# SuperScientificSoftwareLaboratory/PanguLU

Hardware: AMD Instinct MI355X
Metric: numeric factorisation GFLOP/s (pangulu_gstrf, R64) (higher is better)
Workload: dtype f64

## Files before the change

pangulu_amd/csrc/platform/pg_hip_backend.h:

```cpp
#pragma once

struct DiagAux
{
    u32 *d_cp = nullptr;
    u16 *d_ri = nullptr;
    u32 *d_vi = nullptr;
    u32 nnz = 0;
    u32 brow = 0;
};

struct Ring
{
    static const int NSEG = 32;
    std::vector<int> pending;
    size_t seg_bytes = 0;
    char *h = nullptr, *d = nullptr;
    hipEvent_t ev[NSEG];
    bool used[NSEG];
    int cur = 0;
};

struct EventPair
{
    hipEvent_t a, b;
    int cls;
    int split_cls;
    double split_frac;
    unsigned long long tag[3];
};

#define PG_FLOP_WORDS 48

struct Backend
{
    bool ready = false;
    int device = 0;
    hipStream_t stream = nullptr;
    bool bulk_streams_masked = false;
    hipStream_t stream2 = nullptr;
    hipStream_t stream3 = nullptr;
    hipEvent_t ev_fork = nullptr, ev_join = nullptr, ev_fork3 = nullptr, ev_join3 = nullptr;
    hipStream_t stream_front = nullptr;
    hipEvent_t ev_front_fork = nullptr, ev_front_join = nullptr;
    long long opt_front_fork = 1;
    bool getrf_join_pending = false;
    hipStream_t stream_rec = nullptr;
    hipEvent_t ev_rec_fork = nullptr, ev_rec = nullptr;
    std::atomic<bool> rec_dirty{false};
    hipStream_t stream_bg = nullptr;
    hipEvent_t ev_bg_fork = nullptr, ev_bg_done = nullptr;
    hipStream_t stream_early = nullptr;
    bool bg_active = false;
    std::unordered_set<const void *> bg_tiles;
    long long opt_background_updates = 1;
    long long opt_front_stages = 2;
    long long opt_front_min_wgs = 2048;
    long long opt_front_unit = 1;
    long long opt_tiles_stages = 2;
    long long opt_tiles_unit = 1;
    unsigned long long front_workgroups = 0, general_workgroups = 0;
    long long opt_records_stream = 1;
    int nb_cfg = 0;
    unsigned long long generation = 0;
    long long opt_host_mirror = 1;
    long long opt_dense_permille = 2;
    long long opt_profile = 0;
    long long opt_assume_independent = 0;
    long long opt_getrf_strict = 0;
    long long opt_count_flops = 1;
    long long opt_group_chunk = 8;
    long long opt_small_launch_tasks = 2048;
    long long opt_trsm_dense_permille = 5;
    long long opt_two_streams = 1;
    double mfma_flops_executed = 0;
    Ring ring;
    unsigned *d_progress = nullptr;
    size_t progress_next = 0;
    unsigned long long chase_launches = 0, chase_solves = 0;
    unsigned long long zgetrf_tasks = 0;
    unsigned long long *d_flops = nullptr;
    val_t *getrf_scratch = nullptr;
    int getrf_scratch_slots = 0;
    std::unordered_map<const void *, DiagAux> diag_aux;
    pangulu_hip_stats_t stats;
    std::vector<EventPair> pending_events;
    std::vector<hipEvent_t> event_pool;
    std::mutex mutex;
};

Backend B;

struct Recorder
{
    int mode = 0;
    bool valid = false;
    const void *owner = nullptr;
    unsigned long long signature = 0;
    std::vector<std::function<void()>> ops;
    std::vector<std::function<void()>> prologue;
    bool in_prologue = false;
    std::vector<hipEvent_t> early_events;
    struct Seg
    {
        char *h, *d, *twin;
        size_t cap;
    };
    std::vector<Seg> segs;
    size_t descriptor_bytes = 0;
    bool pack = false;
    struct Tail
    {
        int seg;
        size_t used;
    };
    std::vector<Tail> tails;
    int nb = 0;
    unsigned long long generation = 0;
    pangulu_hip_stats_t stats_before, stats_delta;
    unsigned long long wgs_before[4] = {0, 0, 0, 0}, wgs_delta[4] = {0, 0, 0, 0};
};
Recorder REC;

#define PROGRESS_WORDS 8192
struct PendingGetrf
{
    bool active = false, hold = false;
    int nb = 0;
    size_t take = 0;
    const void *d_tasks = nullptr;
    unsigned *d_progress = nullptr;
    std::vector<const double *> images;
    std::function<void()> plain;
    std::function<void()> post;
};
PendingGetrf PEND;
inline void flush_pending_getrf()
{
    if (!PEND.active || PEND.hold)
        return;
    PEND.active = false;
    PEND.plain();
    PEND.post();
    PEND.plain = nullptr;
    PEND.post = nullptr;
}

inline void flush_pending_getrf_locked();

template <class T>
inline T rec_xl(T v)
{
    if constexpr (std::is_pointer<T>::value)
    {
        const char *p = reinterpret_cast<const char *>(v);
        for (const Recorder::Seg &sg : REC.segs)
            if (p >= sg.d && p < sg.d + sg.cap)
                return reinterpret_cast<T>(const_cast<char *>(sg.twin + (p - sg.d)));
    }
    return v;
}

template <class K, class... A>
inline void pg_launch(K kernel, dim3 grid, dim3 block, size_t shmem, hipStream_t st, A... args)
{
    flush_pending_getrf();
    if (REC.mode != 0)
    {
        auto targs = std::make_tuple(rec_xl(args)...);
        (REC.in_prologue ? REC.prologue : REC.ops).emplace_back([=]()
                             { std::apply([&](auto... a)
                                          { hipLaunchKernelGGL(kernel, grid, block, (unsigned)shmem, st, a...); },
                                          targs); });
        if (REC.mode == 2)
            return;
    }
    hipLaunchKernelGGL(kernel, grid, block, (unsigned)shmem, st, args...);
}
#define PG_LAUNCH(kernel_, grid_, block_, shmem_, stream_, ...) pg_launch(kernel_, grid_, block_, shmem_, stream_, __VA_ARGS__)

inline void pg_event_record(hipEvent_t e, hipStream_t s)
{
    flush_pending_getrf();
    if (REC.mode != 0)
        (REC.in_prologue ? REC.prologue : REC.ops).emplace_back([e, s]() { HIP_CHECK(hipEventRecord(e, s)); });
    if (REC.mode != 2)
        HIP_CHECK(hipEventRecord(e, s));
}
inline void pg_stream_wait(hipStream_t s, hipEvent_t e)
{
    flush_pending_getrf();
    if (REC.mode != 0)
        REC.ops.emplace_back([e, s]() { HIP_CHECK(hipStreamWaitEvent(s, e, 0)); });
    if (REC.mode != 2)
        HIP_CHECK(hipStreamWaitEvent(s, e, 0));
}

inline void flush_pending_getrf_locked()
{
    if (!PEND.active)
        return;
    std::lock_guard<std::mutex> g(B.mutex);
    flush_pending_getrf();
}

void ensure_ready()
{
    if (B.ready)
        return;
    int ndev = 0;
    hipError_t e = hipGetDeviceCount(&ndev);
    if (e != hipSuccess || ndev <= 0)
    {
        fprintf(stderr, "[PanguLU-AMD ERROR] no HIP device available (%s); the GPU_HIP platform has no CPU fallback\n",
                e == hipSuccess ? "device count is 0" : hipGetErrorString(e));
        exit(EXIT_FAILURE);
    }
    HIP_CHECK(hipSetDevice(B.device));
    {
        long reserved = 0;
        if (const char *e = getenv("PANGULU_HIP_RESERVED_CUS"))
            reserved = atol(e);
        hipDeviceProp_t prop;
        HIP_CHECK(hipGetDeviceProperties(&prop, B.device));
        const int ncu = prop.multiProcessorCount;
        if (reserved > 0 && reserved < ncu / 2 && ncu % 32 == 0)
        {
            std::vector<uint32_t> mask((size_t)ncu / 32, 0xFFFFFFFFu);
            for (int i = ncu - (int)reserved; i < ncu; i++)
                mask[(size_t)i / 32] &= ~(1u << (i % 32));
            HIP_CHECK(hipExtStreamCreateWithCUMask(&B.stream, (uint32_t)mask.size(), mask.data()));
            HIP_CHECK(hipExtStreamCreateWithCUMask(&B.stream2, (uint32_t)mask.size(), mask.data()));
            B.bulk_streams_masked = true;
        }
        else
        {
            HIP_CHECK(hipStreamCreateWithFlags(&B.stream, hipStreamNonBlocking));
            HIP_CHECK(hipStreamCreateWithFlags(&B.stream2, hipStreamNonBlocking));
        }
    }
    HIP_CHECK(hipStreamCreateWithFlags(&B.stream_front, hipStreamNonBlocking));
    HIP_CHECK(hipEventCreateWithFlags(&B.ev_front_fork, hipEventDisableTiming));
    HIP_CHECK(hipEventCreateWithFlags(&B.ev_front_join, hipEventDisableTiming));
    if (const char *e = getenv("PANGULU_HIP_FRONT_FORK"))
        B.opt_front_fork = atol(e);
    HIP_CHECK(hipEventCreateWithFlags(&B.ev_fork, hipEventDisableTiming));
    HIP_CHECK(hipEventCreateWithFlags(&B.ev_join, hipEventDisableTiming));
    HIP_CHECK(hipStreamCreateWithFlags(&B.stream3, hipStreamNonBlocking));
    HIP_CHECK(hipEventCreateWithFlags(&B.ev_fork3, hipEventDisableTiming));
    HIP_CHECK(hipEventCreateWithFlags(&B.ev_join3, hipEventDisableTiming));
    HIP_CHECK(hipStreamCreateWithFlags(&B.stream_rec, hipStreamNonBlocking));
    HIP_CHECK(hipEventCreateWithFlags(&B.ev_rec_fork, hipEventDisableTiming));
    HIP_CHECK(hipEventCreateWithFlags(&B.ev_rec, hipEventDisableTiming));
    if (const char *e = getenv("PANGULU_HIP_RECORDS_STREAM"))
        B.opt_records_stream = atol(e);
    HIP_CHECK(hipStreamCreateWithFlags(&B.stream_early, hipStreamNonBlocking));
    HIP_CHECK(hipStreamCreateWithFlags(&B.stream_bg, hipStreamNonBlocking));
    HIP_CHECK(hipEventCreateWithFlags(&B.ev_bg_fork, hipEventDisableTiming));
    HIP_CHECK(hipEventCreateWithFlags(&B.ev_bg_done, hipEventDisableTiming));
    if (const char *e = getenv("PANGULU_HIP_BACKGROUND_UPDATES"))
        B.opt_background_updates = atol(e);
    if (const char *e = getenv("PANGULU_HIP_FRONT_STAGES"))
        B.opt_front_stages = atol(e);
    if (const char *e = getenv("PANGULU_HIP_FRONT_UNIT"))
        B.opt_front_unit = atol(e);
    if (const char *e = getenv("PANGULU_HIP_FRONT_MIN_WGS"))
        B.opt_front_min_wgs = atol(e);
    if (const char *e = getenv("PANGULU_HIP_TILES_STAGES"))
        B.opt_tiles_stages = atol(e);
    if (const char *e = getenv("PANGULU_HIP_GROUP_CHUNK"))
        B.opt_group_chunk = atol(e);
    if (const char *e = getenv("PANGULU_HIP_TILES_UNIT"))
        B.opt_tiles_unit = atol(e);
    if (const char *e = getenv("PANGULU_HIP_DENSE_PERMILLE"))
        B.opt_dense_permille = atol(e);
    if (const char *e = getenv("PANGULU_HIP_TRSM_DENSE_PERMILLE"))
        B.opt_trsm_dense_permille = atol(e);
    if (const char *e = getenv("PANGULU_HIP_SMALL_LAUNCH_TASKS"))
        B.opt_small_launch_tasks = atol(e);
    B.ring.seg_bytes = (size_t)8 << 20;
    HIP_CHECK(hipHostMalloc((void **)&B.ring.h, B.ring.seg_bytes * Ring::NSEG, hipHostMallocNonCoherent | hipHostMallocMapped));
    HIP_CHECK(hipHostGetDevicePointer((void **)&B.ring.d, B.ring.h, 0));
    for (int i = 0; i < Ring::NSEG; i++)
    {
        HIP_CHECK(hipEventCreateWithFlags(&B.ring.ev[i], hipEventDisableTiming));
        B.ring.used[i] = false;
    }
    HIP_CHECK(hipMalloc((void **)&B.d_flops, sizeof(unsigned long long) * PG_FLOP_WORDS));
    HIP_CHECK(hipMemset(B.d_flops, 0, sizeof(unsigned long long) * PG_FLOP_WORDS));
    memset(&B.stats, 0, sizeof(B.stats));
    B.ready = true;
}

struct Segment
{
    char *h, *d;
    size_t cap, used;
    int index;
    int rec_idx = -1;
    size_t rec_off = 0;
    template <typename T>
    T *alloc(size_t count, T **dev)
    {
        size_t off = (used + 15) & ~(size_t)15;
        if (off + sizeof(T) * count > cap)
            return nullptr;
        used = off + sizeof(T) * count;
        *dev = reinterpret_cast<T *>(d + off);
        return reinterpret_cast<T *>(h + off);
    }
};

double g_host_seconds[6] = {0, 0, 0, 0, 0, 0};
struct HostTimer
{
    int k;
    std::chrono::steady_clock::time_point t0;
    explicit HostTimer(int k_) : k(k_), t0(std::chrono::steady_clock::now()) {}
    ~HostTimer() { g_host_seconds[k] += std::chrono::duration<double>(std::chrono::steady_clock::now() - t0).count(); }
};

void release_pending_segments(hipStream_t on = nullptr)
{
    Ring &r = B.ring;
    for (int i : r.pending)
    {
        HIP_CHECK(hipEventRecord(r.ev[i], on ? on : B.stream));
        r.used[i] = true;
    }
    r.pending.clear();
}

void join_records(hipStream_t s)
{
    if (!B.rec_dirty.load(std::memory_order_acquire))
        return;
    pg_stream_wait(s, B.ev_rec);
    if (s == B.stream)
        B.rec_dirty.store(false, std::memory_order_release);
}

void join_background(hipStream_t s)
{
    if (!B.bg_active)
        return;
    pg_stream_wait(s, B.ev_bg_done);
    if (s == B.stream)
    {
        B.bg_active = false;
        B.bg_tiles.clear();
    }
}

Segment acquire_segment(size_t want = 0)
{
    Ring &r = B.ring;
    if (REC.mode != 0)
    {
        const size_t min_room = want ? std::min(r.seg_bytes, (want + 4096 + 65535) & ~(size_t)65535) : ((size_t)2 << 20);
        for (size_t k = REC.tails.size(); k-- > 0;)
        {
            const Recorder::Tail t = REC.tails[k];
            const Recorder::Seg &sg = REC.segs[(size_t)t.seg];
            if (sg.cap - t.used < min_room)
                continue;
            REC.tails.erase(REC.tails.begin() + (long)k);
            Segment s;
            s.h = sg.h + t.used;
            s.d = sg.d + t.used;
            s.cap = sg.cap - t.used;
            s.used = 0;
            s.index = -2;
            s.rec_idx = t.seg;
            s.rec_off = t.used;
            return s;
        }
        const size_t bytes = std::min(r.seg_bytes, std::max(min_room, (size_t)4 << 20));
        char *h = nullptr, *d = nullptr, *twin = nullptr;
        HIP_CHECK(hipHostMalloc((void **)&h, bytes, hipHostMallocNonCoherent | hipHostMallocMapped));
        HIP_CHECK(hipHostGetDevicePointer((void **)&d, h, 0));
        HIP_CHECK(hipMalloc((void **)&twin, bytes));
        REC.segs.push_back(Recorder::Seg{h, d, twin, bytes});
        REC.descriptor_bytes += bytes;
        Segment s;
        s.h = h;
        s.d = d;
        s.cap = bytes;
        s.used = 0;
        s.index = -2;
        s.rec_idx = (int)REC.segs.size() - 1;
        s.rec_off = 0;
        return s;
    }
    int i = r.cur;
    r.cur = (r.cur + 1) % Ring::NSEG;
    if (r.used[i])
    {
        HostTimer ht(4);
        HIP_CHECK(hipEventSynchronize(r.ev[i]));
    }
    Segment s;
    s.h = r.h + (size_t)i * r.seg_bytes;
    s.d = r.d + (size_t)i * r.seg_bytes;
    s.cap = r.seg_bytes;
    s.used = 0;
    s.index = i;
    return s;
}

void commit_segment(Segment &s)
{
    if (s.index >= 0)
        B.ring.pending.push_back(s.index);
    else if (s.index == -2 && REC.mode != 0)
    {
        const size_t used = s.rec_off + ((s.used + 255) & ~(size_t)255);
        if (used + ((size_t)64 << 10) <= REC.segs[(size_t)s.rec_idx].cap)
            REC.tails.push_back(Recorder::Tail{s.rec_idx, used});
    }
}
// ... 177 lines not shown
```

pangulu_amd/csrc/platform/pg_hip_front.h:

```cpp
#pragma once

#define FR_TILE 128
#define FR_KS 16
#define FR_LDA 144
#define FR_STAGE_DOUBLES (FR_KS * FR_LDA + FR_TILE * FR_KS)
#define FR_THREADS 512

typedef const char __attribute__((address_space(1))) *fr_gptr;
typedef void __attribute__((address_space(3))) *fr_lptr;

template <int STAGES, bool PREFETCH>
__global__ __launch_bounds__(FR_THREADS, (STAGES <= 2 ? 4 : 2)) void ssssm_front_f64_kernel(const SsssmTaskD *__restrict__ tasks, int nb, const SsssmWorkD *__restrict__ work,
                                                                     unsigned long long *__restrict__ product_counter, unsigned unit)
{
    __shared__ __align__(16) double lds[STAGES * FR_STAGE_DOUBLES];
    const int tiles = nb / FR_TILE;
    const unsigned bid = logical_block_id(unit ? unit : (unsigned)(tiles * tiles));
    const SsssmWorkD G = work[bid];
    const int tile = (int)G.tile;
    const int tid = threadIdx.x, lane = tid & 63;
    const int wave = __builtin_amdgcn_readfirstlane(tid >> 6);
    const int M0 = (tile % tiles) * FR_TILE, N0 = (tile / tiles) * FR_TILE;
    const int wm = (wave & 1) * 64, wn = (wave >> 1) * 32;
    const int l15 = lane & 15, l4 = lane >> 4;
    const int ntask = (int)(G.task_end - G.task_begin);
    const int steps_shift = nb == 256 ? 4 : 3;
    const int steps_per_task = 1 << steps_shift;
    const int T = ntask << steps_shift;
    const SsssmTaskD *my_tasks = tasks + G.task_begin;

    const unsigned a_voff = (unsigned)lane * 16u;
    const int bc = lane >> 3, bj = lane & 7;
    unsigned b_voff[2];
#pragma unroll
    for (int par = 0; par < 2; par++)
        b_voff[par] = ((unsigned)bc * (unsigned)nb + 2u * (unsigned)(bj ^ ((4 * par + (bc >> 1)) & 7))) * 8u;

    auto issue = [&](int st)
    {
        const int t = st >> steps_shift, k0 = (st & (steps_per_task - 1)) * FR_KS;
        const fr_gptr pa = (fr_gptr)reinterpret_cast<const char *>(my_tasks[t].a.val);
        const fr_gptr pb = (fr_gptr)reinterpret_cast<const char *>(my_tasks[t].b.val);
        double *stage = lds + (st % STAGES) * FR_STAGE_DOUBLES;
#pragma unroll
        for (int h = 0; h < 2; h++)
        {
            const int k = wave + 8 * h;
            const fr_gptr src = dg_scalar_base(pa + ((size_t)(k0 + k) * nb + M0) * 8) + a_voff;
            __builtin_amdgcn_global_load_lds((const void __attribute__((address_space(1))) *)src, (fr_lptr)(stage + k * FR_LDA), 16, 0, 0);
        }
#pragma unroll
        for (int h = 0; h < 2; h++)
        {
            const int g = wave + 8 * h;
            const fr_gptr src = dg_scalar_base(pb + ((size_t)(N0 + 8 * g) * nb + k0) * 8) + b_voff[wave & 1];
            __builtin_amdgcn_global_load_lds((const void __attribute__((address_space(1))) *)src, (fr_lptr)(stage + FR_KS * FR_LDA + g * 128), 16, 0, 0);
        }
    };

    double __attribute__((address_space(1))) *C = (double __attribute__((address_space(1))) *)reinterpret_cast<double *>(G.cdense);
    const unsigned c_voff = ((unsigned)l4 * (unsigned)nb + (unsigned)l15) * 8u;
#define FR_C(ni_, mi_, r_)                                                                           \
    (*(double __attribute__((address_space(1))) *)(dg_scalar_base((const char __attribute__((address_space(1))) *)C +                    \
                                                                  ((size_t)(N0 + wn + (ni_) * 16 + 4 * (r_)) * nb + M0 + wm) * 8) + \
                                                   dg_lane_offset(c_voff) + (mi_) * 128))
#ifndef FR_PRELOAD
#define FR_PRELOAD 1
#endif
    const bool preload = FR_PRELOAD && !G.atomic && T > 0;
    v4f64 acc[2][4];
#pragma unroll
    for (int ni = 0; ni < 2; ni++)
#pragma unroll
        for (int mi = 0; mi < 4; mi++)
        {
            if (preload)
            {
#pragma unroll
                for (int r = 0; r < 4; r++)
                    acc[ni][mi][r] = FR_C(ni, mi, r);
            }
            else
                acc[ni][mi] = (v4f64){0.0, 0.0, 0.0, 0.0};
        }

#pragma unroll
    for (int p = 0; p < STAGES - 1; p++)
        if (p < T)
            issue(p);

    const int a_frag = l4 * FR_LDA + wm + l15;
    int b_frag[2][2];
#pragma unroll
    for (int ni = 0; ni < 2; ni++)
    {
        const int n = wn + ni * 16 + l15;
        b_frag[ni][0] = FR_KS * FR_LDA + n * 16 + (l4 & 1);
        b_frag[ni][1] = (n >> 1) & 7;
    }

    for (int st = 0; st < T; st++)
    {
        const int ahead = min(STAGES - 2, T - 1 - st);
        if (STAGES >= 4 && ahead >= 2)
            asm volatile("s_waitcnt vmcnt(8)" ::: "memory");
        else if (STAGES >= 3 && ahead >= 1)
            asm volatile("s_waitcnt vmcnt(4)" ::: "memory");
        else
            asm volatile("s_waitcnt vmcnt(0)" ::: "memory");
        __builtin_amdgcn_s_barrier();
        if (st + STAGES - 1 < T)
            issue(st + STAGES - 1);
        const double *sA = lds + (st % STAGES) * FR_STAGE_DOUBLES;
#if PG_PLANES > 1
        const bool add = my_tasks[st >> steps_shift].sign < 0;
#endif
#if PG_PLANES > 1
#define FR_MFMA(ni_, mi_, fb_, fa_)                                                                                        \
    if (add)                                                                                                                \
        acc[ni_][mi_] = __builtin_amdgcn_mfma_f64_16x16x4f64(fb_, fa_, acc[ni_][mi_], 0, 0, 0);                          \
    else                                                                                                                    \
        acc[ni_][mi_] = __builtin_amdgcn_mfma_f64_16x16x4f64(fb_, fa_, acc[ni_][mi_], 0, 0, DG_NEG_A);
#else
#define FR_MFMA(ni_, mi_, fb_, fa_) acc[ni_][mi_] = __builtin_amdgcn_mfma_f64_16x16x4f64(fb_, fa_, acc[ni_][mi_], 0, 0, DG_NEG_A);
#endif
#define FR_READ(fa_, fb_, kq_)                                                                        \
    {                                                                                                 \
        _Pragma("unroll") for (int mi = 0; mi < 4; mi++)(fa_)[mi] = sA[a_frag + (kq_) * 4 * FR_LDA + mi * 16]; \
        _Pragma("unroll") for (int ni = 0; ni < 2; ni++)(fb_)[ni] = sA[b_frag[ni][0] + 2 * ((2 * (kq_) + (l4 >> 1)) ^ b_frag[ni][1])]; \
    }
        if (PREFETCH)
        {
            double fa[2][4], fb[2][2];
            FR_READ(fa[0], fb[0], 0)
#pragma unroll
            for (int kq = 0; kq < FR_KS / 4; kq++)
            {
                if (kq + 1 < FR_KS / 4)
                    FR_READ(fa[(kq + 1) & 1], fb[(kq + 1) & 1], kq + 1)
#pragma unroll
                for (int ni = 0; ni < 2; ni++)
#pragma unroll
                    for (int mi = 0; mi < 4; mi++)
                    {
                        FR_MFMA(ni, mi, fb[kq & 1][ni], fa[kq & 1][mi])
                    }
            }
        }
        else
        {
#pragma unroll
            for (int kq = 0; kq < FR_KS / 4; kq++)
            {
                double fa[4], fb[2];
                FR_READ(fa, fb, kq)
#pragma unroll
                for (int ni = 0; ni < 2; ni++)
#pragma unroll
                    for (int mi = 0; mi < 4; mi++)
                    {
                        FR_MFMA(ni, mi, fb[ni], fa[mi])
                    }
            }
        }
#undef FR_READ
#undef FR_MFMA
    }
    if (product_counter && lane == 0 && T)
        atomicAdd(product_counter, (unsigned long long)(8 * T));

    if (preload)
    {
#pragma unroll
        for (int ni = 0; ni < 2; ni++)
#pragma unroll
            for (int mi = 0; mi < 4; mi++)
#pragma unroll
                for (int r = 0; r < 4; r++)
                    FR_C(ni, mi, r) = acc[ni][mi][r];
        return;
    }
#pragma unroll
    for (int ni = 0; ni < 2; ni++)
    {
        if (G.atomic)
        {
#pragma unroll
            for (int mi = 0; mi < 4; mi++)
#pragma unroll
                for (int r = 0; r < 4; r++)
                    atomicAdd((double *)&FR_C(ni, mi, r), acc[ni][mi][r]);
            continue;
        }
        double old[4][4];
#pragma unroll
        for (int mi = 0; mi < 4; mi++)
#pragma unroll
            for (int r = 0; r < 4; r++)
                old[mi][r] = FR_C(ni, mi, r);
#pragma unroll
        for (int mi = 0; mi < 4; mi++)
#pragma unroll
            for (int r = 0; r < 4; r++)
                FR_C(ni, mi, r) = old[mi][r] + acc[ni][mi][r];
    }
#undef FR_C
}

#define TL_WINDOW 16
#ifndef TL_MARK
#define TL_PROBE_DECL
#define TL_MARK(i)
#define TL_PROBE_STEP
#define TL_PROBE_FLUSH
#endif
#ifndef TL_ITEM
#define TL_ITEM_DECL
#define TL_ITEM(i)
#define TL_ITEM_COUNT
#endif
#define TV_STEPS (TL_WINDOW * 16)
__global__ __launch_bounds__(FR_THREADS, 4) void ssssm_tilesv_f64_kernel(const SsssmTaskD *__restrict__ tasks, int nb, const SsssmWorkD *__restrict__ work,
                                                                          unsigned long long *__restrict__ product_counter, unsigned unit)
{
    __shared__ __align__(16) double lds[2 * FR_STAGE_DOUBLES];
    __shared__ unsigned long long s_spa[TV_STEPS], s_spb[TV_STEPS];
    __shared__ u32 s_step[TV_STEPS];
    __shared__ u32 s_cnt[FR_THREADS / 64];
#if PG_PLANES > 1
    __shared__ double s_sign[TL_WINDOW];
#endif
    const int tiles = nb / FR_TILE;
    const unsigned bid = logical_block_id(unit ? unit : (unsigned)(tiles * tiles));
    const SsssmWorkD G = work[bid];
    const int tile = (int)G.tile;
    const int tid = threadIdx.x, lane = tid & 63;
    const int wave = __builtin_amdgcn_readfirstlane(tid >> 6);
    const int M0 = (tile % tiles) * FR_TILE, N0 = (tile / tiles) * FR_TILE;
    const int wr = wave & 1, wc = wave >> 1;
    const int l15 = lane & 15, l4 = lane >> 4;
    const int ntask = (int)(G.task_end - G.task_begin);
    const int nslab = nb / FR_KS;
    const SsssmTaskD *my_tasks = tasks + G.task_begin;

    const unsigned a_voff = (unsigned)lane * 16u;
    const int a_piece = lane >> 3;
    const int bc = lane >> 3, bj = lane & 7;
    const unsigned b_voff = ((unsigned)bc * (unsigned)nb + 2u * (unsigned)(bj ^ ((4 * (wave & 1) + (bc >> 1)) & 7))) * 8u;

    v4f64 acc[2][4];
#pragma unroll
    for (int ni = 0; ni < 2; ni++)
#pragma unroll
        for (int mi = 0; mi < 4; mi++)
            acc[ni][mi] = (v4f64){0.0, 0.0, 0.0, 0.0};
    unsigned touched = 0, nprod = 0;

    const int a_frag = l4 * FR_LDA + wr * 16 + l15;
    int b_frag[2][2];
#pragma unroll
    for (int ni = 0; ni < 2; ni++)
    {
        const int n = (wc + 4 * ni) * 16 + l15;
        b_frag[ni][0] = FR_KS * FR_LDA + n * 16 + (l4 & 1);
        b_frag[ni][1] = (n >> 1) & 7;
    }
    const bool all_live = G.pad_ != 0;
    const int slab_shift = nb == 256 ? 4 : 3;

    auto uniform64 = [&](unsigned long long v) -> fr_gptr
    { return (fr_gptr)(((unsigned long long)(unsigned)__builtin_amdgcn_readfirstlane((int)(v >> 32)) << 32) | (unsigned)__builtin_amdgcn_readfirstlane((int)v)); };
    auto issue = [&](unsigned w, fr_gptr pa, fr_gptr pb, int stage_no)
    {
        const unsigned ab = w & 0xFFu, bb = (w >> 8) & 0xFFu;
        const int k0 = (int)((w >> 16) & 15u) * FR_KS;
        double *stage = lds + stage_no * FR_STAGE_DOUBLES;
        const bool a_live = (ab >> a_piece) & 1u;
#pragma unroll
        for (int h = 0; h < 2; h++)
        {
            const int k = wave + 8 * h;
            const unsigned off = a_live ? (unsigned)(((k0 + k) * nb + M0) * 8) + a_voff : 0u;
            __builtin_amdgcn_global_load_lds((const void __attribute__((address_space(1))) *)(dg_scalar_base(pa) + off), (fr_lptr)(stage + k * FR_LDA), 16, 0, 0);
        }
#pragma unroll
        for (int h = 0; h < 2; h++)
        {
            const int g = wave + 8 * h;
            if (!((bb >> (g >> 1)) & 1u))
                continue;
            const unsigned off = (unsigned)(((N0 + 8 * g) * nb + k0) * 8) + b_voff;
            __builtin_amdgcn_global_load_lds((const void __attribute__((address_space(1))) *)(dg_scalar_base(pb) + off), (fr_lptr)(stage + FR_KS * FR_LDA + g * 128), 16, 0, 0);
        }
    };

    double __attribute__((address_space(1))) *C = (double __attribute__((address_space(1))) *)reinterpret_cast<double *>(G.cdense);
    const unsigned c_voff = ((unsigned)l4 * (unsigned)nb + (unsigned)l15) * 8u;
#define TL_C(ni_, mi_, r_)                                                                           \
    (*(double __attribute__((address_space(1))) *)(dg_scalar_base((const char __attribute__((address_space(1))) *)C +                    \
                                                                  ((size_t)(N0 + (wc + 4 * (ni_)) * 16 + 4 * (r_)) * nb + M0 + wr * 16) * 8) + \
                                                   dg_lane_offset(c_voff) + (mi_) * 256))
    unsigned pre = 0;
    const bool may_preload = !G.atomic && ntask <= TL_WINDOW;

    int stage_head = 0;
    TL_ITEM_DECL
    TL_ITEM_COUNT
    for (int win0 = 0; win0 < ntask; win0 += TL_WINDOW)
    {
        __syncthreads();
        int T;
        if (all_live)
        {
            T = min(TL_WINDOW, ntask - win0) * nslab;
            if (tid < T)
            {
                const int t_ = tid >> slab_shift;
                const SsssmTaskD &Tm = my_tasks[win0 + t_];
                s_step[tid] = ((unsigned)t_ << 20) | ((unsigned)(tid & (nslab - 1)) << 16) | 0xFFFFu;
                s_spa[tid] = (unsigned long long)reinterpret_cast<const double *>(Tm.a.val);
                s_spb[tid] = (unsigned long long)reinterpret_cast<const double *>(Tm.b.val);
#if PG_PLANES > 1
                if ((tid & (nslab - 1)) == 0)
                    s_sign[t_] = Tm.sign;
#endif
            }
            __syncthreads();
        }
        else
        {
            unsigned v = 0;
            unsigned long long pa_v = 0, pb_v = 0;
            const int t_ = tid >> 4, s_ = tid & 15;
            if (tid < TL_WINDOW * 16 && win0 + t_ < ntask && s_ < nslab)
            {
                const SsssmTaskD &Tm = my_tasks[win0 + t_];
                const double *pa_ = reinterpret_cast<const double *>(Tm.a.val), *pb_ = reinterpret_cast<const double *>(Tm.b.val);
                pa_v = (unsigned long long)pa_;
                pb_v = (unsigned long long)pb_;
                unsigned ab_, bb_ = 0;
                if (Tm.has_map)
                {
                    ab_ = ((unsigned)Tm.amap[s_] >> (M0 / 16)) & 0xFFu;
                    bb_ = ((unsigned)Tm.bmap_t[s_] >> (N0 / 16)) & 0xFFu;
                }
                else
                {
                    ab_ = ((unsigned)mirror_map(pa_, nb)[s_] >> (M0 / 16)) & 0xFFu;
                    const uint4 mb_ = *reinterpret_cast<const uint4 *>(mirror_map(pb_, nb) + N0 / 16);
                    const unsigned w_[4] = {mb_.x, mb_.y, mb_.z, mb_.w};
#pragma unroll
                    for (int c_ = 0; c_ < 8; c_++)
                        bb_ |= (((w_[c_ >> 1] >> (16 * (c_ & 1))) >> s_) & 1u) << c_;
                }
                if (ab_ && bb_ && (!G.slab_mask || ((G.slab_mask >> s_) & 1u)))
                    v = (bb_ << 8) | ab_ | ((unsigned)s_ << 16) | ((unsigned)t_ << 20);
#if PG_PLANES > 1
                if (s_ == 0)
                    s_sign[t_] = Tm.sign;
#endif
            }
            const unsigned long long bal = __ballot(v != 0);
            TL_ITEM(0)
            if (lane == 0)
                s_cnt[wave] = (u32)__builtin_popcountll(bal);
            __syncthreads();
            unsigned at = (unsigned)__builtin_popcountll(bal & ((1ull << lane) - 1ull)), all = 0;
#pragma unroll
            for (int w_i = 0; w_i < FR_THREADS / 64; w_i++)
            {
                const unsigned c_ = s_cnt[w_i];
                at += w_i < wave ? c_ : 0u;
                all += c_;
            }
            if (v)
            {
                s_step[at] = v;
                s_spa[at] = pa_v;
                s_spb[at] = pb_v;
            }
            __syncthreads();
            T = __builtin_amdgcn_readfirstlane((int)all);
            TL_ITEM(1)
        }
        if (T == 0)
            continue;

        if (may_preload)
        {
            unsigned m = 0;
            if (all_live)
                m = 0xFFu;
            else
            {
                for (int e = lane; e < T; e += 64)
                {
                    const unsigned w = s_step[e];
                    const unsigned ab = w & 0xFFu, bb = (w >> 8) & 0xFFu;
                    const unsigned a4 = ((ab >> wr) & 1u) | (((ab >> (2 + wr)) & 1u) << 1) | (((ab >> (4 + wr)) & 1u) << 2) | (((ab >> (6 + wr)) & 1u) << 3);
                    if ((bb >> wc) & 1u)
                        m |= a4;
                    if ((bb >> (wc + 4)) & 1u)
                        m |= a4 << 4;
                }
#pragma unroll
                for (int off = 32; off > 0; off >>= 1)
                    m |= (unsigned)__shfl_xor((int)m, off, 64);
            }
            pre = (unsigned)__builtin_amdgcn_readfirstlane((int)m);
#pragma unroll
            for (int ni = 0; ni < 2; ni++)
#pragma unroll
                for (int mi = 0; mi < 4; mi++)
                    if ((pre >> (4 * ni + mi)) & 1u)
                    {
#pragma unroll
                        for (int r = 0; r < 4; r++)
                            acc[ni][mi][r] = TL_C(ni, mi, r);
                    }
        }
        TL_ITEM(2)
        unsigned wC = (unsigned)__builtin_amdgcn_readfirstlane((int)s_step[0]), wN = 0;
        fr_gptr paN = uniform64(s_spa[0]), pbN = uniform64(s_spb[0]);
        issue(wC, paN, pbN, stage_head);
        TL_ITEM(3)
        if (T > 1)
        {
            wN = (unsigned)__builtin_amdgcn_readfirstlane((int)s_step[1]);
            paN = uniform64(s_spa[1]);
            pbN = uniform64(s_spb[1]);
        }
        TL_PROBE_DECL
        for (int st = 0; st < T; st++)
        {
            TL_MARK(6)
            TL_PROBE_STEP
            const int e2 = min(st + 2, T - 1);
            const unsigned v_w = s_step[e2];
            const unsigned long long v_pa = s_spa[e2], v_pb = s_spb[e2];
            asm volatile("s_waitcnt vmcnt(0)" ::: "memory");
            TL_MARK(0)
            __builtin_amdgcn_s_barrier();
            TL_MARK(1)
            const unsigned w2 = (unsigned)__builtin_amdgcn_readfirstlane((int)v_w);
            const fr_gptr pa2 = uniform64(v_pa), pb2 = uniform64(v_pb);
            const double *sA = lds + ((stage_head + st) & 1) * FR_STAGE_DOUBLES;
            const unsigned ab = wC & 0xFFu, bb = (wC >> 8) & 0xFFu;
            const unsigned a4 = ((ab >> wr) & 1u) | (((ab >> (2 + wr)) & 1u) << 1) | (((ab >> (4 + wr)) & 1u) << 2) | (((ab >> (6 + wr)) & 1u) << 3);
            const unsigned b2 = ((bb >> wc) & 1u) | (((bb >> (wc + 4)) & 1u) << 1);
            const bool live = a4 && b2;
#if PG_PLANES > 1
            const bool add = s_sign[wC >> 20] < 0;
#endif
#define TV_READ(buf_, kq_)                                                                            \
    {                                                                                                 \
        _Pragma("unroll") for (int mi = 0; mi < 4; mi++) fa[buf_][mi] = sA[a_frag + (kq_) * 4 * FR_LDA + mi * 32]; \
        _Pragma("unroll") for (int ni = 0; ni < 2; ni++) fb[buf_][ni] = sA[b_frag[ni][0] + 2 * ((2 * (kq_) + (l4 >> 1)) ^ b_frag[ni][1])]; \
    }
            double fa[2][4], fb[2][2];
#define TV_PIECE2(ni_, mi_)                                                                                                            \
    if ((m8 >> ((mi_) + 4 * (ni_))) & 1u)                                                                                              \
    {                                                                                                                                   \
        TV_ONE(0, ni_, mi_)                                                                                                             \
        TV_ONE(1, ni_, mi_)                                                                                                             \
    }
#if PG_PLANES > 1
#define TV_ONE(buf_, ni_, mi_)                                                                                                          \
    if (add)                                                                                                                            \
        acc[ni_][mi_] = __builtin_amdgcn_mfma_f64_16x16x4f64(fb[buf_][ni_], fa[buf_][mi_], acc[ni_][mi_], 0, 0, 0);                     \
    else                                                                                                                                \
        acc[ni_][mi_] = __builtin_amdgcn_mfma_f64_16x16x4f64(fb[buf_][ni_], fa[buf_][mi_], acc[ni_][mi_], 0, 0, DG_NEG_A);
#else
#define TV_ONE(buf_, ni_, mi_) acc[ni_][mi_] = __builtin_amdgcn_mfma_f64_16x16x4f64(fb[buf_][ni_], fa[buf_][mi_], acc[ni_][mi_], 0, 0, DG_NEG_A);
#endif
#define TV_PAIR                                                                            \
    {                                                                                      \
        TV_PIECE2(0, 0) TV_PIECE2(0, 1) TV_PIECE2(0, 2) TV_PIECE2(0, 3)                    \
        TV_PIECE2(1, 0) TV_PIECE2(1, 1) TV_PIECE2(1, 2) TV_PIECE2(1, 3)                    \
    }
            unsigned m8 = 0;
            if (live)
            {
                m8 = ((b2 & 1u) ? a4 : 0u) | ((b2 & 2u) ? (a4 << 4) : 0u);
                nprod += (unsigned)__builtin_popcount(m8);
                touched |= m8;
                TV_READ(0, 0)
                TV_READ(1, 1)
                TV_PAIR
            }
            TL_MARK(2)
            if (st + 1 < T)
                issue(wN, paN, pbN, (stage_head + st + 1) & 1);
            TL_MARK(3)
            if (live)
            {
                TV_READ(0, 2)
                TV_READ(1, 3)
                TV_PAIR
            }
#undef TV_PIECE2
#undef TV_ONE
#undef TV_PAIR
#undef TV_READ
            wC = wN;
            wN = w2;
            paN = pa2;
            pbN = pb2;
            TL_MARK(4)
        }
        TL_PROBE_FLUSH
        stage_head = (stage_head + T) & 1;
        TL_ITEM(4)
    }
    if (product_counter && lane == 0 && nprod)
        atomicAdd(product_counter, (unsigned long long)nprod);

    if (pre)
    {
#pragma unroll
        for (int ni = 0; ni < 2; ni++)
#pragma unroll
            for (int mi = 0; mi < 4; mi++)
                if ((pre >> (4 * ni + mi)) & 1u)
                {
#pragma unroll
                    for (int r = 0; r < 4; r++)
                        TL_C(ni, mi, r) = acc[ni][mi][r];
                }
        touched = 0;
    }
#pragma unroll
    for (int ni = 0; ni < 2; ni++)
    {
        const unsigned t4 = (touched >> (4 * ni)) & 0xFu;
        if (!t4)
            continue;
        if (G.atomic)
        {
#pragma unroll
            for (int mi = 0; mi < 4; mi++)
            {
                if (!((t4 >> mi) & 1u))
                    continue;
#pragma unroll
                for (int r = 0; r < 4; r++)
                    if (acc[ni][mi][r] != 0.0)
                        atomicAdd((double *)&TL_C(ni, mi, r), acc[ni][mi][r]);
            }
            continue;
        }
        double old[4][4];
#pragma unroll
        for (int mi = 0; mi < 4; mi++)
#pragma unroll
            for (int r = 0; r < 4; r++)
                old[mi][r] = ((t4 >> mi) & 1u) ? TL_C(ni, mi, r) : 0.0;
#pragma unroll
        for (int mi = 0; mi < 4; mi++)
        {
            if (!((t4 >> mi) & 1u))
                continue;
// ... 12 lines not shown
```

pangulu_amd/csrc/platform/pg_hip_launch_ssssm.h:

```cpp
#pragma once

#define DG_TILE_HOST 128
size_t launch_chunk_tasks()
{
    static const size_t chunk = []()
    {
        const char *e = getenv("PANGULU_HIP_LAUNCH_CHUNK");
        long v = e ? atol(e) : 0;
        return v > 0 ? (size_t)v : ~(size_t)0;
    }();
    return chunk;
}

void launch_ssssm(int nb, task_t **list, size_t n, bool background = false)
{
    if (n == 0)
        return;
    HostTimer ht(0);
    hipStream_t const ms = background ? B.stream_bg : B.stream;
    const bool dense_ok = dense_mode_available(nb);
    static std::unordered_set<const void *> bg_earlier;
    bg_earlier.clear();
    size_t i = 0;
    while (i < n)
    {
        bool bg_hazard = false;
        const size_t chunk_begin = i;
        const size_t per_task = sizeof(SsssmTaskD) * (1 + PG_PLANES * PG_PLANES) + sizeof(SsssmGroupD) * (1 + PG_PLANES) +
                                sizeof(SsssmWorkD) * 8 * PG_PLANES;
        const size_t fixed_part = 64 * 4 * PG_PLANES * (sizeof(SsssmGroupD) + 4 * sizeof(SsssmWorkD)) + 4096;
        Segment seg = acquire_segment(std::min(n - i, launch_chunk_tasks()) * per_task + fixed_part + 65536);
        size_t max_tasks = (seg.cap - fixed_part) / per_task;
        size_t take = std::min(n - i, std::min(max_tasks, launch_chunk_tasks()));
        SsssmTaskD *d_tasks_s, *d_tasks_d;
        SsssmGroupD *d_groups_s, *d_groups_d;
        SsssmTaskD *tasks_s = seg.alloc<SsssmTaskD>(take, &d_tasks_s);
        SsssmTaskD *tasks_d = seg.alloc<SsssmTaskD>(take * PG_PLANES * PG_PLANES, &d_tasks_d);
        const int tiles_per_dim = nb >= DG_TILE_HOST ? nb / DG_TILE_HOST : 1;
        const unsigned ksplit = (nb <= 256 && nb % 64 == 0 && take * (size_t)(tiles_per_dim * tiles_per_dim) <= 64) ? 4u : 1u;
        SsssmGroupD *groups_s = seg.alloc<SsssmGroupD>(take, &d_groups_s);
        SsssmGroupD *groups_d = seg.alloc<SsssmGroupD>(take * ksplit * PG_PLANES, &d_groups_d);
        static std::vector<unsigned short> live_k;
        live_k.assign(take * 4 * PG_PLANES * PG_PLANES, 0);
        static std::vector<unsigned char> full_t;
        full_t.assign(take * PG_PLANES * PG_PLANES, 0);
        SsssmWorkD *d_work, *d_work_f;
        SsssmWorkD *work = seg.alloc<SsssmWorkD>(take * ksplit * 4 * PG_PLANES, &d_work);
        SsssmWorkD *work_f = seg.alloc<SsssmWorkD>(take * 4 * PG_PLANES, &d_work_f);
        if (!tasks_s || !tasks_d || !groups_s || !groups_d || !work || !work_f)
        {
            fprintf(stderr, "[PanguLU-AMD ERROR] descriptor staging segment too small\n");
            exit(EXIT_FAILURE);
        }
        size_t ns = 0, nd = 0, gs = 0, gd = 0, nd_updates = 0;
        double bytes_s = 0, bytes_d = 0;
        size_t end = i + take;
        while (i < end)
        {
            slot_t *dst = canon_dst(list[i]->opdst);
            size_t j = i;
            while (j < end && canon_dst(list[j]->opdst) == dst)
                j++;
            const bool diag = dst->brow_pos == dst->bcol_pos;
            SsssmGroupD G;
            memset(&G, 0, sizeof(G));
            u32 nnz_c;
            slot_t *up = nullptr, *lo = dst;
            if (diag)
            {
                diag_halves(dst, &up, &lo);
                nnz_c = host_nnz(lo, nb) + host_nnz(up, nb);
            }
            else
            {
                nnz_c = host_nnz(dst, nb);
            }
#if defined(PG_DENSE_UPDATES)
            double *cm = nullptr;
            const size_t jobs_before = MP.to_densify.size() + MP.to_sparsify.size() + MP.early.size();
            if (dense_ok)
            {
                bool want = mirror_is_ahead(dst);
                for (size_t t = i; t < j && !want; t++)
                    want = is_heavy_update(host_nnz(list[t]->op1, nb), host_nnz(list[t]->op2, nb), nb);
                if (want)
                    cm = current_mirror(dst, nb);
                if (cm)
                {
                    block_state(dst, nb).sparse_current = false;
                    G.cdense = reinterpret_cast<val_t *>(cm);
                }
            }
            if (!cm)
            {
                require_sparse(dst, nb);
                block_state(dst, nb).written = true;
            }
            if (background && !bg_earlier.empty() && MP.to_densify.size() + MP.to_sparsify.size() + MP.early.size() != jobs_before &&
                bg_earlier.count(block_key_any(dst)))
                bg_hazard = true;
#endif
            if (!G.cdense)
            {
                G.c = BlkView{lo->d_columnpointer, lo->d_rowindex, lo->d_value};
                if (diag)
                {
                    const DiagAux &aux = get_diag_aux(up, nb);
                    G.ucp = aux.d_cp;
                    G.uri = aux.d_ri;
                    G.uvi = aux.d_vi;
                    G.uval = up->d_value;
                }
            }
            size_t s0 = ns;
#if defined(PG_DENSE_UPDATES)
            struct Heavy
            {
                SsssmTaskD T;
                unsigned short live[4];
                unsigned char full;
            };
            static thread_local std::vector<Heavy> heavy;
            heavy.clear();
#endif
            for (size_t t = i; t < j; t++)
            {
                if (t + PREFETCH_SLOTS_AHEAD < n)
                    prefetch_task_slots(list[t + PREFETCH_SLOTS_AHEAD]);
                if (t + PREFETCH_DETAILS_AHEAD < n)
                    prefetch_task_details(list[t + PREFETCH_DETAILS_AHEAD], nb);
                slot_t *a = list[t]->op1, *b = list[t]->op2;
                SsssmTaskD T;
                memset(&T, 0, sizeof(T));
                T.a = BlkView{a->d_columnpointer, a->d_rowindex, a->d_value};
                T.b = BlkView{b->d_columnpointer, b->d_rowindex, b->d_value};
                T.sign = 1.0;
                T.count = 1;
                u32 na = host_nnz(a, nb), nbz = host_nnz(b, nb);
                double by = (SV + 2) * ((double)na + nbz) + (2 * SV + 2) * (double)nnz_c + 12.0 * (nb + 1);
                bool on_mfma = false;
#if defined(PG_DENSE_UPDATES)
                if (G.cdense && is_heavy_update(na, nbz, nb))
                {
                    double *am = current_mirror(a, nb);
                    double *bm = am ? current_mirror(b, nb) : nullptr;
                    if (am && bm)
                    {
                        T.a.val = reinterpret_cast<val_t *>(am);
                        T.b.val = reinterpret_cast<val_t *>(bm);
                        on_mfma = true;
                    }
                }
                if (on_mfma)
                {
                    Heavy H;
                    H.T = T;
                    const BlockState *sa = MP.blocks.find(block_key(a)), *sb = MP.blocks.find(block_key(b));
                    for (int tl = 0; tl < 4; tl++)
                        H.live[tl] = tl >= tiles_per_dim * tiles_per_dim ? (unsigned short)0
                                     : (sa && sb && sa->occ_valid && sb->occ_valid)
                                         ? (unsigned short)(sa->occ_a[tl % tiles_per_dim] & sb->occ_b[tl / tiles_per_dim])
                                         : (unsigned short)0xFFFF;
                    H.full = 0;
                    if (sa && sb && sa->occ_valid && sb->occ_valid)
                    {
                        H.T.has_map = 1;
                        memcpy(H.T.amap, sa->occ_map, sizeof(H.T.amap));
                        memcpy(H.T.bmap_t, sb->occ_map_t, sizeof(H.T.bmap_t));
                        const int nslab = nb / 16;
                        const unsigned pm = nb >= 128 ? 0xFFu : ((1u << nslab) - 1u);
                        for (int tl = 0; tl < tiles_per_dim * tiles_per_dim; tl++)
                        {
                            const int tm = tl % tiles_per_dim, tn = tl / tiles_per_dim;
                            bool all = true;
                            for (int sl = 0; sl < nslab && all; sl++)
                                all = (((unsigned)H.T.amap[sl] >> (8 * tm)) & pm) == pm && (((unsigned)H.T.bmap_t[sl] >> (8 * tn)) & pm) == pm;
                            if (all)
                                H.full |= (unsigned char)(1u << tl);
                        }
                    }
                    heavy.push_back(H);
                    bytes_d += by;
                    nd_updates++;
                }
#endif
                if (!on_mfma)
                {
                    tasks_s[ns++] = T;
                    bytes_s += by;
                }
            }
            size_t chunk = (size_t)(B.opt_group_chunk > 0 ? B.opt_group_chunk : 1 << 30);
// ... 272 lines not shown
```

Baseline: 48820.

## Factor front GEMM body into device function and hoist task pointer loads

Moves the front SSSSM kernel body into a reusable device function that loads the next task's A/B pointers and sign one step ahead instead of inside the issue path, and by default issues the next stage's global-to-LDS loads after the first MFMA slice rather than right after the barrier. The tiles kernel now hands all-live groups to this front path instead of its own all-live window code. An environment switch can turn off ksplit. The intent is to take descriptor loads off the critical path and overlap load issue with compute, at the cost of more registers and changed scheduling.

```diff
diff --git a/pangulu_amd/csrc/platform/pg_hip_backend.h b/pangulu_amd/csrc/platform/pg_hip_backend.h
--- a/pangulu_amd/csrc/platform/pg_hip_backend.h
+++ b/pangulu_amd/csrc/platform/pg_hip_backend.h
@@ -55,6 +55,7 @@
     long long opt_background_updates = 1;
     long long opt_front_stages = 2;
     long long opt_front_min_wgs = 2048;
+    long long opt_ksplit = 1;
     long long opt_front_unit = 1;
     long long opt_tiles_stages = 2;
     long long opt_tiles_unit = 1;
@@ -265,6 +266,8 @@
         B.opt_front_unit = atol(e);
     if (const char *e = getenv("PANGULU_HIP_FRONT_MIN_WGS"))
         B.opt_front_min_wgs = atol(e);
+    if (const char *e = getenv("PANGULU_HIP_KSPLIT"))
+        B.opt_ksplit = atol(e);
     if (const char *e = getenv("PANGULU_HIP_TILES_STAGES"))
         B.opt_tiles_stages = atol(e);
     if (const char *e = getenv("PANGULU_HIP_GROUP_CHUNK"))
diff --git a/pangulu_amd/csrc/platform/pg_hip_front.h b/pangulu_amd/csrc/platform/pg_hip_front.h
--- a/pangulu_amd/csrc/platform/pg_hip_front.h
+++ b/pangulu_amd/csrc/platform/pg_hip_front.h
@@ -9,14 +9,19 @@
 typedef const char __attribute__((address_space(1))) *fr_gptr;
 typedef void __attribute__((address_space(3))) *fr_lptr;
 
-template <int STAGES, bool PREFETCH>
-__global__ __launch_bounds__(FR_THREADS, (STAGES <= 2 ? 4 : 2)) void ssssm_front_f64_kernel(const SsssmTaskD *__restrict__ tasks, int nb, const SsssmWorkD *__restrict__ work,
-                                                                     unsigned long long *__restrict__ product_counter, unsigned unit)
+#ifndef FR_ISSUE_FIRST
+#define FR_ISSUE_FIRST 0
+#endif
+#define FR_ORDER (FR_ISSUE_FIRST ? 0 : 1)
+#ifndef FR_PRELOAD
+#define FR_PRELOAD 1
+#endif
+
+template <int STAGES, bool PREFETCH, int ORDER>
+__device__ __forceinline__ void fr_front_item(double *lds, const SsssmTaskD *__restrict__ tasks, int nb, const SsssmWorkD &G,
+                                              unsigned long long *__restrict__ product_counter)
 {
-    __shared__ __align__(16) double lds[STAGES * FR_STAGE_DOUBLES];
     const int tiles = nb / FR_TILE;
-    const unsigned bid = logical_block_id(unit ? unit : (unsigned)(tiles * tiles));
-    const SsssmWorkD G = work[bid];
     const int tile = (int)G.tile;
     const int tid = threadIdx.x, lane = tid & 63;
     const int wave = __builtin_amdgcn_readfirstlane(tid >> 6);
@@ -36,11 +41,9 @@
     for (int par = 0; par < 2; par++)
         b_voff[par] = ((unsigned)bc * (unsigned)nb + 2u * (unsigned)(bj ^ ((4 * par + (bc >> 1)) & 7))) * 8u;
 
-    auto issue = [&](int st)
-    {
-        const int t = st >> steps_shift, k0 = (st & (steps_per_task - 1)) * FR_KS;
-        const fr_gptr pa = (fr_gptr)reinterpret_cast<const char *>(my_tasks[t].a.val);
-        const fr_gptr pb = (fr_gptr)reinterpret_cast<const char *>(my_tasks[t].b.val);
+    auto issue = [&](int st, fr_gptr pa, fr_gptr pb)
+    {
+        const int k0 = (st & (steps_per_task - 1)) * FR_KS;
         double *stage = lds + (st % STAGES) * FR_STAGE_DOUBLES;
 #pragma unroll
         for (int h = 0; h < 2; h++)
@@ -64,9 +67,6 @@
     (*(double __attribute__((address_space(1))) *)(dg_scalar_base((const char __attribute__((address_space(1))) *)C +                    \
                                                                   ((size_t)(N0 + wn + (ni_) * 16 + 4 * (r_)) * nb + M0 + wm) * 8) + \
                                                    dg_lane_offset(c_voff) + (mi_) * 128))
-#ifndef FR_PRELOAD
-#define FR_PRELOAD 1
-#endif
     const bool preload = FR_PRELOAD && !G.atomic && T > 0;
     v4f64 acc[2][4];
 #pragma unroll
@@ -84,10 +84,20 @@
                 acc[ni][mi] = (v4f64){0.0, 0.0, 0.0, 0.0};
         }
 
+    fr_gptr pa_rq = nullptr, pb_rq = nullptr;
+    if (T > 0)
+    {
+        pa_rq = (fr_gptr)reinterpret_cast<const char *>(my_tasks[0].a.val);
+        pb_rq = (fr_gptr)reinterpret_cast<const char *>(my_tasks[0].b.val);
+    }
+#if PG_PLANES > 1
+    bool add = T > 0 && my_tasks[0].sign < 0;
+#endif
+
 #pragma unroll
     for (int p = 0; p < STAGES - 1; p++)
         if (p < T)
-            issue(p);
+            issue(p, pa_rq, pb_rq);
 
     const int a_frag = l4 * FR_LDA + wm + l15;
     int b_frag[2][2];
@@ -101,6 +111,19 @@
 
     for (int st = 0; st < T; st++)
     {
+        const int rq = st + STAGES - 1;
+        fr_gptr pa_nx = pa_rq, pb_nx = pb_rq;
+        if (((rq + 1) & (steps_per_task - 1)) == 0 && rq + 1 < T)
+        {
+            const SsssmTaskD &Tn = my_tasks[(rq + 1) >> steps_shift];
+            pa_nx = (fr_gptr)reinterpret_cast<const char *>(Tn.a.val);
+            pb_nx = (fr_gptr)reinterpret_cast<const char *>(Tn.b.val);
+        }
+#if PG_PLANES > 1
+        bool add_nx = add;
+        if (((st + 1) & (steps_per_task - 1)) == 0 && st + 1 < T)
+            add_nx = my_tasks[(st + 1) >> steps_shift].sign < 0;
+#endif
         const int ahead = min(STAGES - 2, T - 1 - st);
         if (STAGES >= 4 && ahead >= 2)
             asm volatile("s_waitcnt vmcnt(8)" ::: "memory");
@@ -109,12 +132,10 @@
         else
             asm volatile("s_waitcnt vmcnt(0)" ::: "memory");
         __builtin_amdgcn_s_barrier();
-        if (st + STAGES - 1 < T)
-            issue(st + STAGES - 1);
+        const bool request = rq < T;
+        if (ORDER == 0 && request)
+            issue(rq, pa_rq, pb_rq);
         const double *sA = lds + (st % STAGES) * FR_STAGE_DOUBLES;
-#if PG_PLANES > 1
-        const bool add = my_tasks[st >> steps_shift].sign < 0;
-#endif
 #if PG_PLANES > 1
 #define FR_MFMA(ni_, mi_, fb_, fa_)                                                                                        \
     if (add)                                                                                                                \
@@ -129,6 +150,9 @@
         _Pragma("unroll") for (int mi = 0; mi < 4; mi++)(fa_)[mi] = sA[a_frag + (kq_) * 4 * FR_LDA + mi * 16]; \
         _Pragma("unroll") for (int ni = 0; ni < 2; ni++)(fb_)[ni] = sA[b_frag[ni][0] + 2 * ((2 * (kq_) + (l4 >> 1)) ^ b_frag[ni][1])]; \
     }
+#define FR_REQUEST_BEHIND(kq_)                   \
+    if (ORDER == 1 && (kq_) == 0 && request)     \
+        issue(rq, pa_rq, pb_rq);
         if (PREFETCH)
         {
             double fa[2][4], fb[2][2];
@@ -145,6 +169,7 @@
                     {
                         FR_MFMA(ni, mi, fb[kq & 1][ni], fa[kq & 1][mi])
                     }
+                FR_REQUEST_BEHIND(kq)
             }
         }
         else
@@ -161,10 +186,17 @@
                     {
                         FR_MFMA(ni, mi, fb[ni], fa[mi])
                     }
-            }
-        }
+                FR_REQUEST_BEHIND(kq)
+            }
+        }
+#undef FR_REQUEST_BEHIND
 #undef FR_READ
 #undef FR_MFMA
+        pa_rq = pa_nx;
+        pb_rq = pb_nx;
+#if PG_PLANES > 1
+        add = add_nx;
+#endif
     }
     if (product_counter && lane == 0 && T)
         atomicAdd(product_counter, (unsigned long long)(8 * T));
@@ -205,6 +237,17 @@
                 FR_C(ni, mi, r) = old[mi][r] + acc[ni][mi][r];
     }
 #undef FR_C
+}
+
+template <int STAGES, bool PREFETCH>
+__global__ __launch_bounds__(FR_THREADS, (STAGES <= 2 ? 4 : 2)) void ssssm_front_f64_kernel(const SsssmTaskD *__restrict__ tasks, int nb, const SsssmWorkD *__restrict__ work,
+                                                                     unsigned long long *__restrict__ product_counter, unsigned unit)
+{
+    __shared__ __align__(16) double lds[STAGES * FR_STAGE_DOUBLES];
+    const int tiles = nb / FR_TILE;
+    const unsigned bid = logical_block_id(unit ? unit : (unsigned)(tiles * tiles));
+    const SsssmWorkD G = work[bid];
+    fr_front_item<STAGES, PREFETCH, FR_ORDER>(lds, tasks, nb, G, product_counter);
 }
 
 #define TL_WINDOW 16
@@ -239,6 +282,11 @@
     const int M0 = (tile % tiles) * FR_TILE, N0 = (tile / tiles) * FR_TILE;
     const int wr = wave & 1, wc = wave >> 1;
     const int l15 = lane & 15, l4 = lane >> 4;
+    if (G.pad_ != 0)
+    {
+        fr_front_item<2, true, FR_ORDER>(lds, tasks, nb, G, product_counter);
+        return;
+    }
     const int ntask = (int)(G.task_end - G.task_begin);
     const int nslab = nb / FR_KS;
     const SsssmTaskD *my_tasks = tasks + G.task_begin;
@@ -265,8 +313,6 @@
         b_frag[ni][0] = FR_KS * FR_LDA + n * 16 + (l4 & 1);
         b_frag[ni][1] = (n >> 1) & 7;
     }
-    const bool all_live = G.pad_ != 0;
-    const int slab_shift = nb == 256 ? 4 : 3;
 
     auto uniform64 = [&](unsigned long long v) -> fr_gptr
     { return (fr_gptr)(((unsigned long long)(unsigned)__builtin_amdgcn_readfirstlane((int)(v >> 32)) << 32) | (unsigned)__builtin_amdgcn_readfirstlane((int)v)); };
@@ -310,24 +356,6 @@
     {
         __syncthreads();
         int T;
-        if (all_live)
-        {
-            T = min(TL_WINDOW, ntask - win0) * nslab;
-            if (tid < T)
-            {
-                const int t_ = tid >> slab_shift;
-                const SsssmTaskD &Tm = my_tasks[win0 + t_];
-                s_step[tid] = ((unsigned)t_ << 20) | ((unsigned)(tid & (nslab - 1)) << 16) | 0xFFFFu;
-                s_spa[tid] = (unsigned long long)reinterpret_cast<const double *>(Tm.a.val);
-                s_spb[tid] = (unsigned long long)reinterpret_cast<const double *>(Tm.b.val);
-#if PG_PLANES > 1
-                if ((tid & (nslab - 1)) == 0)
-                    s_sign[t_] = Tm.sign;
-#endif
-            }
-            __syncthreads();
-        }
-        else
         {
             unsigned v = 0;
             unsigned long long pa_v = 0, pb_v = 0;
@@ -389,24 +417,19 @@
         if (may_preload)
         {
             unsigned m = 0;
-            if (all_live)
-                m = 0xFFu;
-            else
-            {
-                for (int e = lane; e < T; e += 64)
-                {
-                    const unsigned w = s_step[e];
-                    const unsigned ab = w & 0xFFu, bb = (w >> 8) & 0xFFu;
-                    const unsigned a4 = ((ab >> wr) & 1u) | (((ab >> (2 + wr)) & 1u) << 1) | (((ab >> (4 + wr)) & 1u) << 2) | (((ab >> (6 + wr)) & 1u) << 3);
-                    if ((bb >> wc) & 1u)
-                        m |= a4;
-                    if ((bb >> (wc + 4)) & 1u)
-                        m |= a4 << 4;
-                }
-#pragma unroll
-                for (int off = 32; off > 0; off >>= 1)
-                    m |= (unsigned)__shfl_xor((int)m, off, 64);
-            }
+            for (int e = lane; e < T; e += 64)
+            {
+                const unsigned w = s_step[e];
+                const unsigned ab = w & 0xFFu, bb = (w >> 8) & 0xFFu;
+                const unsigned a4 = ((ab >> wr) & 1u) | (((ab >> (2 + wr)) & 1u) << 1) | (((ab >> (4 + wr)) & 1u) << 2) | (((ab >> (6 + wr)) & 1u) << 3);
+                if ((bb >> wc) & 1u)
+                    m |= a4;
+                if ((bb >> (wc + 4)) & 1u)
+                    m |= a4 << 4;
+            }
+#pragma unroll
+            for (int off = 32; off > 0; off >>= 1)
+                m |= (unsigned)__shfl_xor((int)m, off, 64);
             pre = (unsigned)__builtin_amdgcn_readfirstlane((int)m);
 #pragma unroll
             for (int ni = 0; ni < 2; ni++)
diff --git a/pangulu_amd/csrc/platform/pg_hip_launch_ssssm.h b/pangulu_amd/csrc/platform/pg_hip_launch_ssssm.h
--- a/pangulu_amd/csrc/platform/pg_hip_launch_ssssm.h
+++ b/pangulu_amd/csrc/platform/pg_hip_launch_ssssm.h
@@ -37,7 +37,7 @@
         SsssmTaskD *tasks_s = seg.alloc<SsssmTaskD>(take, &d_tasks_s);
         SsssmTaskD *tasks_d = seg.alloc<SsssmTaskD>(take * PG_PLANES * PG_PLANES, &d_tasks_d);
         const int tiles_per_dim = nb >= DG_TILE_HOST ? nb / DG_TILE_HOST : 1;
-        const unsigned ksplit = (nb <= 256 && nb % 64 == 0 && take * (size_t)(tiles_per_dim * tiles_per_dim) <= 64) ? 4u : 1u;
+        const unsigned ksplit = (B.opt_ksplit != 0 && nb <= 256 && nb % 64 == 0 && take * (size_t)(tiles_per_dim * tiles_per_dim) <= 64) ? 4u : 1u;
         SsssmGroupD *groups_s = seg.alloc<SsssmGroupD>(take, &d_groups_s);
         SsssmGroupD *groups_d = seg.alloc<SsssmGroupD>(take * ksplit * PG_PLANES, &d_groups_d);
         static std::vector<unsigned short> live_k;
```

New measurement: 49420, median of 6. +1.2%, better.
